# pierotofy/OpenSplat

Hardware: NVIDIA H100
Metric: fwd_bwd_mpixel_per_s (higher is better)
Workload: dtype f32

## Files before the change

include/gsplat_b200.h:

```cpp
#ifndef GSPLAT_B200_H
#define GSPLAT_B200_H

#include <stddef.h>
#include <stdint.h>

#ifdef __cplusplus
extern "C" {
#endif

#define GSB_TILE 16
#define GSB_ERR_INVALID_ARG (-1)
#define GSB_ERR_WORKSPACE (-2)
#define GSB_ERR_UNSUPPORTED (-3)
#define GSB_RASTER_CLAMP_MAX_ONE 1u
#define GSB_BIN_COUNT_VISIBLE 2

typedef void *gsb_stream_t;

int gsb_version(void);
const char *gsb_last_error(void);

int gsb_sh_forward(int n, int degree, int degrees_to_use, const float *viewdirs, const float *coeffs,
                   float *colors, gsb_stream_t stream);
int gsb_sh_backward(int n, int degree, int degrees_to_use, const float *viewdirs, const float *v_colors,
// ... 54 lines not shown
int gsb_project_backward_activated(int n, const float *means3d, const float *log_scales, float glob_scale,
                                   const float *raw_quats, const float *opacities, const float *viewmat,
                                   const float *projmat, float fx, float fy, int img_h, int img_w,
                                   const int32_t *radii, const float *conics, const float *v_xy,
                                   const float *v_depth, const float *v_conic, const float *v_opacity,
                                   float *v_mean3d, float *v_log_scales, float *v_raw_quats,
                                   float *v_opacity_logits, gsb_stream_t stream);
int gsb_project_backward_activated_acc(int n, const float *means3d, const float *log_scales, float glob_scale,
                                       const float *raw_quats, const float *opacities, const float *viewmat,
                                       const float *projmat, float fx, float fy, int img_h, int img_w,
                                       const int32_t *radii, const float *conics, const float *v_xy,
                                       const float *v_depth, const float *v_conic, const float *v_opacity,
                                       float *v_mean3d, float *v_log_scales, float *v_raw_quats,
                                       float *v_opacity_logits, gsb_stream_t stream);

size_t gsb_cumsum_workspace_bytes(int n);
int gsb_cumsum_tiles_hit(int n, const int32_t *num_tiles_hit, int32_t *cum_tiles_hit, void *workspace,
                         size_t workspace_bytes, gsb_stream_t stream);
int gsb_map_gaussian_to_intersects(int n, int m, const float *xys, const float *depths,
                                   const int32_t *radii, const int32_t *cum_tiles_hit, int tiles_x,
                                   int tiles_y, int64_t *isect_ids, int32_t *gaussian_ids,
                                   gsb_stream_t stream);
size_t gsb_sort_workspace_bytes(int m);
int gsb_sort_intersects(int m, int num_tiles, const int64_t *isect_ids, int64_t *isect_ids_sorted,
                        int32_t *sorted_index, void *workspace, size_t workspace_bytes,
                        gsb_stream_t stream);
int gsb_gather_bin_edges(int m, int num_tiles, const int64_t *isect_ids_sorted,
                         const int32_t *sorted_index, const int32_t *gaussian_ids,
                         int32_t *gaussian_ids_sorted, int32_t *tile_bins, gsb_stream_t stream);

int gsb_bucket_max_tile_len(void);
size_t gsb_bucket_workspace_bytes(int n, int m_capacity, int num_tiles);
int gsb_bucket_tile_ranges(int n, const float *xys, const int32_t *radii, const float *conics, const float *colors,
                           const float *opacities, int cull, int tiles_x, int tiles_y, int m_capacity,
                           int len_capacity, void *workspace, size_t workspace_bytes, int32_t *cum_tiles_hit,
                           int32_t *tile_bins, int32_t *tile_order, int32_t *stats, gsb_stream_t stream);
int gsb_bucket_sort_pack(int n, int m_capacity, int len_capacity, const float *depths, const int32_t *radii,
                         const int32_t *cum_tiles_hit, int cull, int tiles_x, int tiles_y, const int32_t *tile_bins,
                         const int32_t *stats, void *workspace, size_t workspace_bytes, void *records,
                         int32_t *sorted_index, int32_t *gaussian_ids_sorted, gsb_stream_t stream);

size_t gsb_raster_records_bytes(int m);
size_t gsb_raster_grad_rows_bytes(int m);
int gsb_pack_records(int m, const int32_t *gaussian_ids_sorted, const int32_t *sorted_index, const float *xys,
                     const float *conics, const float *colors, const float *opacities, void *records,
                     gsb_stream_t stream);
int gsb_rasterize_forward_packed(int img_h, int img_w, int tiles_x, int tiles_y, int m, const int32_t *tile_bins,
                                 const int32_t *tile_order, const int32_t *bin_stats, const float *background,
                                 void *records, float *out_img, float *final_Ts, int32_t *final_idx,
                                 unsigned flags, gsb_stream_t stream);
int gsb_rasterize_forward_count(int img_h, int img_w, int tiles_x, int tiles_y, int m, const int32_t *tile_bins,
                                const float *background, void *records, float *out_img, float *final_Ts,
                                int32_t *final_idx, unsigned long long *pair_counts, gsb_stream_t stream);
int gsb_rasterize_backward(int img_h, int img_w, int tiles_x, int tiles_y, int n, int m, const int32_t *tile_bins,
                           const int32_t *tile_order, const float *conics, const float *opacities, void *records,
                           const int32_t *cum_tiles_hit, const float *background, const float *final_Ts,
                           const int32_t *final_idx, const float *v_output, const float *v_output_alpha,
                           void *grad_rows, float *v_xy, float *v_conic, float *v_colors, float *v_opacity,
                           unsigned flags, gsb_stream_t stream);

int gsb_mse_loss_grad(long long n, const float *img, const float *target, float *v_img, float *loss_out,
                      float inv_count, gsb_stream_t stream);
int gsb_adam_step(long long n, float *param, const float *grad, float *exp_avg, float *exp_avg_sq, float lr,
                  float beta1, float beta2, float eps, float bias_correction1, float bias_correction2,
                  gsb_stream_t stream);
#define GSB_ADAM_MAX_SEGMENTS 8
typedef struct gsb_adam_segment {
    long long offset, count;
    int row_floats, head_floats;
    float lr_head, lr_rest;
} gsb_adam_segment;
int gsb_adam_step_segments(int num_segments, const gsb_adam_segment *segments, float *param, const float *grad,
                           float *exp_avg, float *exp_avg_sq, float beta1, float beta2, float eps,
                           float bias_correction1, float bias_correction2, gsb_stream_t stream);

int gsb_activate_forward(int n, const float *means, const float *log_scales, const float *raw_quats,
                         const float *opacity_logits, const float *cam_pos, float *scales, float *quats,
                         float *opacities, float *viewdirs, gsb_stream_t stream);
int gsb_activate_backward(int n, const float *scales, const float *raw_quats, const float *opacities,
                          const float *v_scales, const float *v_quats, const float *v_opacities,
                          float *v_log_scales, float *v_raw_quats, float *v_opacity_logits, gsb_stream_t stream);

int gsb_densify_stats_update(int n, const float *v_xy, const int32_t *radii, int img_h, int img_w,
                             float *xys_grad_norm, float *vis_counts, float *max_2d_size, gsb_stream_t stream);
int gsb_densify_stats_init(int n, const float *v_xy, const int32_t *radii, int img_h, int img_w,
                           float *xys_grad_norm, float *vis_counts, float *max_2d_size, gsb_stream_t stream);

size_t gsb_densify_workspace_bytes(int n);
int gsb_densify_classify(int n, const float *scales, const float *opacities, const float *xys_grad_norm,
                         const float *vis_counts, const float *max_2d_size, float max_dim,
                         float densify_grad_thresh, float densify_size_thresh, int check_split_screen,
                         float split_screen_size, float cull_alpha_thresh, int check_huge, float cull_scale_thresh,
                         int check_cull_screen, float cull_screen_size, float size_fac, void *workspace,
                         size_t workspace_bytes, int32_t *src_map, int32_t *split_rank, int32_t *counts,
                         gsb_stream_t stream);
int gsb_densify_means_scales(int new_n, int n_splits, const int32_t *src_map, const int32_t *split_rank,
                             const float *samples, const float *means, const float *scales, const float *quats,
                             float size_fac, float *new_means, float *new_scales, gsb_stream_t stream);
int gsb_densify_gather_rows(int new_n, int row_floats, const int32_t *src_map, const float *src, float *dst,
                            int zero_children, gsb_stream_t stream);
int gsb_reset_opacity(int n, float max_logit, float *opacities, float *exp_avg, float *exp_avg_sq,
                      gsb_stream_t stream);

int gsb_ply_row_floats(int sh_bases);
int gsb_pack_ply_rows(int n, int sh_bases, const float *means, const float *features_dc, int dc_stride,
                      const float *features_rest, int rest_stride, const float *opacities, const float *scales,
// ... 34 lines not shown
```

opensplat_b200/capi.py:

```python
import ctypes as C
import os

import torch

_HERE = os.path.dirname(os.path.abspath(__file__))
LIB_PATH = os.environ.get("GSB_LIB") or os.path.join(_HERE, "lib", "libgsplat_b200.so")
_lib = None

_vp, _i, _f, _sz = C.c_void_p, C.c_int, C.c_float, C.c_size_t

_SIGS = {
    "gsb_version": (C.c_int, []),
    "gsb_last_error": (C.c_char_p, []),
    "gsb_sh_forward": (_i, [_i, _i, _i, _vp, _vp, _vp, _vp]),
    "gsb_sh_backward": (_i, [_i, _i, _i, _vp, _vp, _vp, _vp]),
    "gsb_sh_forward_rgb": (_i, [_i, _i, _i, _vp, _vp, _f, _vp, _vp]),
    "gsb_sh_backward_rgb": (_i, [_i, _i, _i, _vp, _vp, _vp, _vp, _vp]),
    "gsb_sh_forward_split": (_i, [_i, _i, _i, _vp, _vp, _vp, _vp, _f, _vp, _vp]),
    "gsb_sh_backward_split": (_i, [_i, _i, _i, _vp, _vp, _vp, _vp, _vp, _vp, _vp]),
    "gsb_sh_forward_rgb_cam": (_i, [_i, _i, _i, _vp, _vp, _vp, _f, _vp, _vp]),
    "gsb_sh_backward_rgb_cam": (_i, [_i, _i, _i, _vp, _vp, _vp, _vp, _vp, _vp]),
    "gsb_sh_forward_rgb_cam_multiview": (_i, [_i, _i, _i, _vp, _i, _vp, _vp, _f, _vp, _vp]),
    "gsb_mask_rgb_grad": (_i, [_i, _vp, _vp, _vp]),
    "gsb_sh_backward_multiview": (_i, [_i, _i, _i, _vp, _i, _vp, _vp, _f, _vp, _vp]),
    "gsb_exchange_gradients": (_i, [_i, _i, _i, _vp, _i, _vp, _vp, _f, _vp, _i, _i, C.c_longlong, _vp, _vp, _vp]),
    "gsb_sh_backward_multiview_cams": (_i, [_i, _i, _i, _vp, _i, _vp, _vp, _f, _vp, _vp]),
    "gsb_exchange_gradients_cams": (_i, [_i, _i, _i, _vp, _i, _vp, _vp, _f, _vp, _i, _i, C.c_longlong, _vp, _vp,
                                         _vp]),
    "gsb_project_forward": (_i, [_i, _vp, _vp, _f, _vp, _vp, _vp, _f, _f, _f, _f, _i, _i, _i, _i, _f,
                                 _vp, _vp, _vp, _vp, _vp, _vp, _vp]),
    "gsb_project_backward": (_i, [_i, _vp, _vp, _f, _vp, _vp, _vp, _f, _f, _f, _f, _i, _i,
                                  _vp, _vp, _vp, _vp, _vp, _vp, _vp, _vp, _vp, _vp]),
    "gsb_project_forward_activated": (_i, [_i, _vp, _vp, _f, _vp, _vp, _vp, _vp, _f, _f, _f, _f, _i, _i, _i, _i, _f,
                                           _vp, _vp, _vp, _vp, _vp, _vp, _vp, _vp]),
    "gsb_project_backward_activated": (_i, [_i, _vp, _vp, _f, _vp, _vp, _vp, _vp, _f, _f, _i, _i,
                                            _vp, _vp, _vp, _vp, _vp, _vp, _vp, _vp, _vp, _vp, _vp]),
    "gsb_project_backward_activated_acc": (_i, [_i, _vp, _vp, _f, _vp, _vp, _vp, _vp, _f, _f, _i, _i,
                                                _vp, _vp, _vp, _vp, _vp, _vp, _vp, _vp, _vp, _vp, _vp]),
    "gsb_cumsum_workspace_bytes": (_sz, [_i]),
    "gsb_cumsum_tiles_hit": (_i, [_i, _vp, _vp, _vp, _sz, _vp]),
    "gsb_map_gaussian_to_intersects": (_i, [_i, _i, _vp, _vp, _vp, _vp, _i, _i, _vp, _vp, _vp]),
    "gsb_sort_workspace_bytes": (_sz, [_i]),
    "gsb_sort_intersects": (_i, [_i, _i, _vp, _vp, _vp, _vp, _sz, _vp]),
    "gsb_gather_bin_edges": (_i, [_i, _i, _vp, _vp, _vp, _vp, _vp, _vp]),
    "gsb_raster_records_bytes": (_sz, [_i]),
    "gsb_raster_grad_rows_bytes": (_sz, [_i]),
    "gsb_pack_records": (_i, [_i, _vp, _vp, _vp, _vp, _vp, _vp, _vp, _vp]),
    "gsb_rasterize_forward_packed": (_i, [_i, _i, _i, _i, _i, _vp, _vp, _vp, _vp, _vp, _vp, _vp, _vp, C.c_uint, _vp]),
    "gsb_rasterize_forward_count": (_i, [_i, _i, _i, _i, _i, _vp, _vp, _vp, _vp, _vp, _vp, _vp, _vp]),
    "gsb_rasterize_backward": (_i, [_i, _i, _i, _i, _i, _i, _vp, _vp, _vp, _vp, _vp, _vp, _vp, _vp, _vp, _vp,
                                    _vp, _vp, _vp, _vp, _vp, _vp, C.c_uint, _vp]),
    "gsb_bucket_max_tile_len": (_i, []),
    "gsb_bucket_workspace_bytes": (_sz, [_i, _i, _i]),
    "gsb_bucket_tile_ranges": (_i, [_i, _vp, _vp, _vp, _vp, _vp, _i, _i, _i, _i, _i, _vp, _sz, _vp, _vp, _vp, _vp, _vp]),
    "gsb_bucket_sort_pack": (_i, [_i, _i, _i, _vp, _vp, _vp, _i, _i, _i, _vp, _vp, _vp, _sz, _vp, _vp, _vp, _vp]),
    "gsb_activate_forward": (_i, [_i, _vp, _vp, _vp, _vp, _vp, _vp, _vp, _vp, _vp, _vp]),
    "gsb_activate_backward": (_i, [_i, _vp, _vp, _vp, _vp, _vp, _vp, _vp, _vp, _vp, _vp]),
    "gsb_densify_stats_update": (_i, [_i, _vp, _vp, _i, _i, _vp, _vp, _vp, _vp]),
    "gsb_densify_stats_init": (_i, [_i, _vp, _vp, _i, _i, _vp, _vp, _vp, _vp]),
    "gsb_densify_workspace_bytes": (_sz, [_i]),
    "gsb_densify_classify": (_i, [_i, _vp, _vp, _vp, _vp, _vp, _f, _f, _f, _i, _f, _f, _i, _f, _i, _f, _f, _vp, _sz,
                                  _vp, _vp, _vp, _vp]),
    "gsb_densify_means_scales": (_i, [_i, _i, _vp, _vp, _vp, _vp, _vp, _vp, _f, _vp, _vp, _vp]),
    "gsb_densify_gather_rows": (_i, [_i, _i, _vp, _vp, _vp, _i, _vp]),
    "gsb_reset_opacity": (_i, [_i, _f, _vp, _vp, _vp, _vp]),
    "gsb_ply_row_floats": (_i, [_i]),
    "gsb_pack_ply_rows": (_i, [_i, _i, _vp, _vp, _i, _vp, _i, _vp, _vp, _vp, _i, _f, C.POINTER(C.c_float), _vp, _vp]),
    "gsb_unpack_ply_rows": (_i, [_i, _i, _vp, _i, _f, C.POINTER(C.c_float), _vp, _vp, _i, _vp, _i, _vp, _vp, _vp, _vp]),
    "gsb_splat_order_keys": (_i, [_i, _vp, _vp, _i, _f, _vp, _vp]),
    "gsb_pack_splat_rows": (_i, [_i, _vp, _vp, _vp, _vp, _i, _vp, _vp, _i, _f, C.POINTER(C.c_float), _vp, _vp]),
    "gsb_ssim_workspace_bytes": (_sz, [_i, _i]),
    "gsb_ssim_l1_loss": (_i, [_i, _i, _vp, _vp, _f, _vp, _vp, _vp, _sz, _vp]),
    "gsb_adam_step": (_i, [C.c_longlong, _vp, _vp, _vp, _vp, _f, _f, _f, _f, _f, _f, _vp]),
    "gsb_adam_step_segments": (_i, [_i, _vp, _vp, _vp, _vp, _vp, _f, _f, _f, _f, _f, _vp]),
    "gsb_mse_loss_grad": (_i, [C.c_longlong, _vp, _vp, _vp, _vp, _f, _vp]),
    "gsb_knn_workspace_bytes": (_sz, [_i]),
    "gsb_knn_mean_dist": (_i, [_i, _vp, _vp, _vp, _sz, _vp]),
    "gsb_resize_area_u8": (_i, [_i, _i, _vp, _i, _i, _vp, _f, _vp]),
    "gsb_undistort_u8": (_i, [_i, _i, _vp, _f, _f, _f, _f, _f, _f, _f, _f, _f, _f, _f, _f, _f, _i, _i, _i, _i, _vp,
                              _vp]),
    "gsb_u8_to_f32_views": (_i, [_i, _vp, _i, _i, _vp, _vp]),
}

ADAM_MAX_SEGMENTS = 8


class AdamSegment(C.Structure):
    _fields_ = [("offset", C.c_longlong), ("count", C.c_longlong), ("row_floats", C.c_int),
                ("head_floats", C.c_int), ("lr_head", C.c_float), ("lr_rest", C.c_float)]
_OPT_SIGS = {}


class GsbError(RuntimeError):
    pass


def lib():
    global _lib
    if _lib is None:
        if not os.path.exists(LIB_PATH):
            raise GsbError(f"{LIB_PATH} not built -- run `python -m opensplat_b200.build` "
                           "(there is no CPU fallback)")
# ... 38 lines not shown
```

opensplat_b200/csrc/bucket.cu:

```cuda
#include "raster_common.cuh"

namespace {

constexpr int CUR_STRIDE = 32;
constexpr int BIN_THREADS = 256;
constexpr int TSCAN_THREADS = 1024;

constexpr int LEN_BUCKETS = 64;
struct BinHeader {
    unsigned ticket_n;
    unsigned ticket_t;
    unsigned done_t;
    int max_len;
    int total;
    int visible;
    int pad0[2];
    int len_hist[LEN_BUCKETS];
    int len_cur[LEN_BUCKETS];
    int pad[120];
};
static_assert(sizeof(BinHeader) == 1024, "header is 1 KB");

__device__ __forceinline__ int len_bucket(int v, int len_capacity) {
    const long long b = (long long)v * LEN_BUCKETS / ((long long)max(len_capacity, 1) + 1);
// ... 16 lines not shown
    if (blk == 0) {
        if (lane == 0) st_state(&state[0], ST_INC | (unsigned)aggregate);
        return 0;
    }
    if (lane == 0) st_state(&state[blk], ST_AGG | (unsigned)aggregate);
    int excl = 0;
    int j = blk - 1;
    while (true) {
        const int idx = j - lane;
        unsigned long long s = ST_INC;
        if (idx >= 0) s = ld_state(&state[idx]);
        const unsigned flag = (unsigned)(s >> 62);
        if (__ballot_sync(0xffffffffu, flag == 0u)) continue;
        const unsigned incm = __ballot_sync(0xffffffffu, flag == 2u);
        int val = (int)(unsigned)(s & ST_VAL);
        if (incm) {
            const int first = __ffs(incm) - 1;
            if (lane > first) val = 0;
            excl += __reduce_add_sync(0xffffffffu, val);
            break;
        }
        excl += __reduce_add_sync(0xffffffffu, val);
        j -= 32;
    }
    if (lane == 0) st_state(&state[blk], ST_INC | (unsigned)(excl + aggregate));
    return excl;
}

__global__ void __launch_bounds__(BIN_THREADS)
bin_count_kernel(int n, const float2 *__restrict__ xys, const int *__restrict__ radii,
                 const float *__restrict__ conics, const float *__restrict__ colors,
                 const float *__restrict__ opacities, int cull, int tiles_x, int tiles_y,
                 int *__restrict__ tile_count, GsbRecord *__restrict__ gattr, int *__restrict__ count_out,
                 int *__restrict__ visible) {
    const int i = blockIdx.x * BIN_THREADS + threadIdx.x;
    const int r = (i < n) ? radii[i] : 0;
    if (visible) {
        const int nvis = __syncthreads_count(r > 0);
        if (threadIdx.x == 0 && nvis > 0) atomicAdd(visible, nvis);
    }
    if (i >= n) return;
    int cnt = 0;
    if (r > 0) {
        const float2 c = xys[i];
        const GsbRecord rec = make_record(c, __ldg(conics + 3 * i), __ldg(conics + 3 * i + 1),
                                          __ldg(conics + 3 * i + 2), __ldg(opacities + i), __ldg(colors + 3 * i),
                                          __ldg(colors + 3 * i + 1), __ldg(colors + 3 * i + 2), 0);
        float4 *dst = reinterpret_cast<float4 *>(gattr + i);
        dst[0] = rec.q0; dst[1] = rec.q1; dst[2] = rec.q2;
        int x0, x1, y0, y1;
        gsb_tile_bbox(c.x, c.y, (float)r, tiles_x, tiles_y, x0, x1, y0, y1);
        for (int ty = y0; ty < y1; ++ty)
            for (int tx = x0; tx < x1; ++tx) {
                if (cull && !extent_slot_mask(c.x, c.y, rec.q1.w, rec.q2.w, (float)(tx * GSB_TILE),
                                              (float)(ty * GSB_TILE)))
                    continue;
                atomicAdd(&tile_count[(size_t)(ty * tiles_x + tx) * CUR_STRIDE], 1);
                ++cnt;
            }
    }
    count_out[i] = cnt;
}

constexpr int GS_IPT = 8;
__global__ void __launch_bounds__(BIN_THREADS)
count_scan_kernel(int n, int *__restrict__ counts_then_cum, unsigned *ticket, unsigned long long *state) {
    __shared__ int sm[BIN_THREADS / 32 + 1];
    __shared__ int s_blk, s_prefix;
    if (threadIdx.x == 0) s_blk = (int)atomicAdd(ticket, 1u);
    __syncthreads();
    const int blk = s_blk;
    const int e0 = (blk * BIN_THREADS + threadIdx.x) * GS_IPT;
    int v[GS_IPT];
    const bool vec = (e0 + GS_IPT <= n) && ((reinterpret_cast<uintptr_t>(counts_then_cum + e0) & 15) == 0);
    if (vec) {
        const int4 a = *reinterpret_cast<const int4 *>(counts_then_cum + e0);
        const int4 b = *reinterpret_cast<const int4 *>(counts_then_cum + e0 + 4);
        v[0] = a.x; v[1] = a.y; v[2] = a.z; v[3] = a.w; v[4] = b.x; v[5] = b.y; v[6] = b.z; v[7] = b.w;
    } else {
#pragma unroll
        for (int k = 0; k < GS_IPT; ++k) v[k] = (e0 + k < n) ? counts_then_cum[e0 + k] : 0;
    }
    int tsum = 0;
#pragma unroll
    for (int k = 0; k < GS_IPT; ++k) tsum += v[k];
    int total;
    int run = block_excl_scan<BIN_THREADS>(tsum, &total, sm);
    if (threadIdx.x < 32) {
        const int p = chained_scan_prefix(state, blk, total);
        if (threadIdx.x == 0) s_prefix = p;
    }
    __syncthreads();
    run += s_prefix;
#pragma unroll
    for (int k = 0; k < GS_IPT; ++k) { run += v[k]; v[k] = run; }
    if (vec) {
        *reinterpret_cast<int4 *>(counts_then_cum + e0) = make_int4(v[0], v[1], v[2], v[3]);
        *reinterpret_cast<int4 *>(counts_then_cum + e0 + 4) = make_int4(v[4], v[5], v[6], v[7]);
    } else {
#pragma unroll
        for (int k = 0; k < GS_IPT; ++k)
            if (e0 + k < n) counts_then_cum[e0 + k] = v[k];
    }
}

}

int gsb_count_scan_blocks(int n) { return gsb_div_up(n > 0 ? n : 1, BIN_THREADS * GS_IPT); }
// ... 23 lines not shown
        const int p = chained_scan_prefix(state, blk, total);
        if (threadIdx.x == 0) s_prefix = p;
    }
    __syncthreads();
    if (t < T) {
        const int e = s_prefix + excl;
        tile_bins[t] = (v > 0) ? make_int2(e, e + v) : make_int2(0, 0);
        tile_count_then_cursor[(size_t)t * CUR_STRIDE] = e;
    }
    if (threadIdx.x == 0) {
        if (s_max > 0) atomicMax(&hdr->max_len, s_max);
        if (blk == nblk - 1) atomicExch(&hdr->total, s_prefix + total);
        __threadfence();
        const unsigned done = atomicAdd(&hdr->done_t, 1u);
        if (done == (unsigned)nblk - 1u) {
            __threadfence();
            const int M = atomicAdd(&hdr->total, 0), mx = atomicAdd(&hdr->max_len, 0);
            stats[0] = M;
            stats[1] = mx;
            stats[2] = (M > m_capacity || mx > len_capacity) ? 1 : 0;
            stats[3] = hdr->visible;
        }
    }
}

__global__ void __launch_bounds__(TSCAN_THREADS)
tile_order_kernel(int T, int len_capacity, BinHeader *hdr, const int2 *__restrict__ tile_bins,
                  int *__restrict__ tile_order) {
    __shared__ int base[LEN_BUCKETS];
    if (threadIdx.x < LEN_BUCKETS) {
        int sfx = 0;
        for (int b = LEN_BUCKETS - 1; b > (int)threadIdx.x; --b) sfx += hdr->len_hist[b];
        base[threadIdx.x] = sfx;
    }
    __syncthreads();
    const int t = blockIdx.x * TSCAN_THREADS + threadIdx.x;
    if (t >= T) return;
    const int2 r = tile_bins[t];
    const int b = len_bucket(r.y - r.x, len_capacity);
    tile_order[base[b] + atomicAdd(&hdr->len_cur[b], 1)] = t;
}

__global__ void __launch_bounds__(256)
bucket_emit_kernel(int n, const GsbRecord *__restrict__ gattr, const float *__restrict__ depths,
                   const int *__restrict__ radii, const int *__restrict__ cum_tiles_hit, int cull, int tiles_x,
                   int tiles_y, int *__restrict__ cursor, unsigned long long *__restrict__ comp,
                   int *__restrict__ gaussian_ids, int *__restrict__ gid_at_pos, const int *__restrict__ stats) {
    if (stats[2]) return;
    const int i = blockIdx.x * blockDim.x + threadIdx.x;
    if (i >= n) return;
    const int r = radii[i];
    if (r <= 0) return;
    const float4 *src = reinterpret_cast<const float4 *>(gattr + i);
    const float4 q0 = src[0];
    const float hx = src[1].w, hy = src[2].w;
    int x0, x1, y0, y1;
    gsb_tile_bbox(q0.x, q0.y, (float)r, tiles_x, tiles_y, x0, x1, y0, y1);
    int k = (i == 0) ? 0 : cum_tiles_hit[i - 1];
    const unsigned long long hi = ((unsigned long long)(unsigned)__float_as_int(depths[i])) << 32;
    for (int ty = y0; ty < y1; ++ty)
        for (int tx = x0; tx < x1; ++tx) {
            if (cull && !extent_slot_mask(q0.x, q0.y, hx, hy, (float)(tx * GSB_TILE), (float)(ty * GSB_TILE)))
                continue;
            const int pos = atomicAdd(&cursor[(size_t)(ty * tiles_x + tx) * CUR_STRIDE], 1);
            comp[pos] = hi | (unsigned)k;
            if (gid_at_pos) gid_at_pos[pos] = i;
            gaussian_ids[k] = i;
            ++k;
        }
}

typedef unsigned long long u64;

constexpr int DS_MIN_BINS = 64, DS_MAX_BINS = 2048;
constexpr int DS_BIN_LIMIT = 32;

constexpr int BITONIC_MAX = 4096;

__device__ __forceinline__ u64 shfl_xor_u64(u64 v, int m) {
    unsigned lo = (unsigned)v, hi = (unsigned)(v >> 32);
    lo = __shfl_xor_sync(0xffffffffu, lo, m);
    hi = __shfl_xor_sync(0xffffffffu, hi, m);
    return ((u64)hi << 32) | lo;
}

__device__ __forceinline__ u64 cex_shfl(u64 v, int j, bool keep_min) {
    const u64 o = shfl_xor_u64(v, j);
    return ((v < o) == keep_min) ? v : o;
}

__device__ __forceinline__ void block64_substages(u64 &a, u64 &b, int base, int lane, int k, int jstart) {
    const int ia = base + lane, ib = ia + 32;
    const bool asc_a = (ia & k) == 0, asc_b = (ib & k) == 0;
    if (jstart >= 32) {
        const bool sw = (a > b) == asc_a;
        const u64 t = sw ? b : a;
        b = sw ? a : b;
        a = t;
    }
#pragma unroll
    for (int j = 16; j >= 1; j >>= 1) {
        if (j > jstart) continue;
        const bool lower = (lane & j) == 0;
        a = cex_shfl(a, j, lower == asc_a);
        b = cex_shfl(b, j, lower == asc_b);
    }
}

template <int ITEMS>
__device__ __forceinline__ void cta_radix_sort_depth(u64 *buf, unsigned (*whist)[256], unsigned *bin_base,
                                                    unsigned *s_flag) {
    const int lane = threadIdx.x & 31, w = threadIdx.x >> 5;
    const int wbase = w * 32 * ITEMS;
    u64 key[ITEMS];
    unsigned rank[ITEMS];
// ... 480 lines not shown
```

opensplat_b200/csrc/raster_bwd.cu:

```cuda
#include "raster_common.cuh"

int gsb_blend_grid(const void *kernel, int num_tiles);

namespace {

__device__ __forceinline__ float rcp_approx(float x) {
    float y;
    asm("rcp.approx.ftz.f32 %0, %1;" : "=f"(y) : "f"(x));
    return y;
}

__device__ __forceinline__ void zero_row(float *grad_rows, int k) {
    float4 *row = reinterpret_cast<float4 *>(grad_rows + (size_t)k * GSB_GRAD_ROW_FLOATS);
    const float4 z = make_float4(0.f, 0.f, 0.f, 0.f);
    row[0] = z; row[1] = z; row[2] = z;
}

constexpr int BWD_MIN_BLOCKS = 6;
template <bool SAT>
__global__ void __launch_bounds__(RK_THREADS, BWD_MIN_BLOCKS)
rasterize_backward_kernel(int img_h, int img_w, int tiles_x, int num_tiles,
                          const int2 *__restrict__ tile_bins, const GsbRecord *__restrict__ records,
                          const float *__restrict__ background, const float *__restrict__ final_Ts,
                          const int *__restrict__ final_idx, const float *__restrict__ v_output,
                          const float *__restrict__ v_output_alpha, float *__restrict__ grad_rows,
                          unsigned *__restrict__ tile_counter, const int *__restrict__ tile_order) {
    __shared__ WarpRing rings[RK_WARPS];
    const int warp = threadIdx.x >> 5, lane = threadIdx.x & 31;
    WarpRing &ring = rings[warp];
    if (lane == 0) {
#pragma unroll
        for (int s = 0; s < RK_STAGES; ++s) mbar_init(&ring.full[s], 1);
        mbar_fence_init();
    }
    __syncwarp();
    const float bg0 = __ldg(background), bg1 = __ldg(background + 1), bg2 = __ldg(background + 2);
    unsigned gchunk = 0;

    while (true) {
        int tile = 0;
        if (lane == 0) tile = (int)atomicAdd(tile_counter, 1u);
        tile = __shfl_sync(0xffffffffu, tile, 0);
        if (tile >= num_tiles) break;
        if (tile_order) tile = __ldg(tile_order + tile);
        const int2 range = tile_bins[tile];
        if (range.y <= range.x) continue;

        const int tx = tile % tiles_x, ty = tile / tiles_x;
        const int X = tx * GSB_TILE + (lane & 15);
        const int Y0 = ty * GSB_TILE + (lane >> 4);
        const float px = (float)X;
        const float tile_x0 = (float)(tx * GSB_TILE), tile_y0 = (float)(ty * GSB_TILE);

        float T[RK_PIX], Bq[RK_PIX];
        const float py0 = (float)Y0;
        float vor[RK_PIX], vog[RK_PIX], vob[RK_PIX];
        int binf[RK_PIX];
        int my_max = -1;
#pragma unroll
        for (int j = 0; j < RK_PIX; ++j) {
            const int Y = Y0 + 2 * j;
            if (X < img_w && Y < img_h) {
                const size_t p = (size_t)Y * img_w + X;
// ... 227 lines not shown
```

opensplat_b200/csrc/raster_common.cuh:

```cuda
#pragma once
#include "gsb_common.cuh"

struct __align__(16) GsbRecord {
    float4 q0, q1, q2;
};
static_assert(sizeof(GsbRecord) == 48, "record must be 48 bytes");

constexpr int RK_WARPS = 4;
constexpr int RK_THREADS = RK_WARPS * 32;
constexpr int RK_PIX = 8;
constexpr int RK_CHUNK = 32;
constexpr int RK_STAGES = 4;

constexpr float GSB_LN2 = 0.6931471805599453f;
constexpr float GSB_LOG2E = 1.4426950408889634f;
constexpr float GSB_SMAX_BIAS = 5.541263545158426f + 1e-3f;

constexpr int GSB_GRAD_ROW_FLOATS = 12;

constexpr int GSB_SAT_BIT0 = 1 << 28;
constexpr int GSB_SAT_MASK = 7 << 28;

struct __align__(128) WarpRing {
    GsbRecord rec[RK_STAGES][RK_CHUNK];
    uint64_t full[RK_STAGES];
};

#ifdef __CUDACC__
__device__ __forceinline__ GsbRecord make_record(float2 xy, float a, float b, float c, float opac, float r,
                                                 float g, float bl, int k) {
    const float lo = (opac > 0.f) ? log2f(opac) : -INFINITY;
    const float smax = fmaxf(0.f, fmaf(lo, GSB_LN2, GSB_SMAX_BIAS));
    const float det = a * c - b * b;
    float hx = INFINITY, hy = INFINITY;
    if (det > 0.f && a > 0.f && c > 0.f) {
        const float s2 = 2.f * smax / det;
        hx = sqrtf(s2 * c) * 1.001f + 0.01f;
        hy = sqrtf(s2 * a) * 1.001f + 0.01f;
    }
    GsbRecord rec;
    rec.q0 = make_float4(xy.x, xy.y, lo, __int_as_float(k));
    rec.q1 = make_float4(0.5f * a, b, 0.5f * c, hx);
    rec.q2 = make_float4(r, g, bl, hy);
    return rec;
}

__device__ __forceinline__ unsigned extent_slot_mask(float cx, float cy, float hx, float hy, float tile_x0,
                                                     float tile_y0) {
    const float gx = cx - tile_x0, gy = cy - tile_y0;
    const float xlo = fmaxf(ceilf(gx - hx), 0.f), xhi = fminf(floorf(gx + hx), 15.f);
    const float ylo = fmaxf(ceilf(gy - hy), 0.f), yhi = fminf(floorf(gy + hy), 15.f);
    if (!(xlo <= xhi) || !(ylo <= yhi)) return 0u;
    const int jlo = (int)ylo >> 1, jhi = (int)yhi >> 1;
    return ((2u << jhi) - 1u) & ~((1u << jlo) - 1u);
}

__device__ __forceinline__ unsigned record_slot_mask(const GsbRecord &r, float tile_x0, float tile_y0) {
    return extent_slot_mask(r.q0.x, r.q0.y, r.q1.w, r.q2.w, tile_x0, tile_y0);
}
#endif
```

opensplat_b200/csrc/raster_fwd.cu:

```cuda
#include "raster_common.cuh"

namespace {

__global__ void __launch_bounds__(256)
pack_records_kernel(int m, const int *__restrict__ gaussian_ids_sorted,
                    const int *__restrict__ sorted_index, const float2 *__restrict__ xys,
                    const float *__restrict__ conics, const float *__restrict__ colors,
                    const float *__restrict__ opacities, GsbRecord *__restrict__ records) {
    const int i = blockIdx.x * blockDim.x + threadIdx.x;
    if (i >= m) return;
    const int g = gaussian_ids_sorted[i];
    const int k = sorted_index ? sorted_index[i] : i;
    const GsbRecord r = make_record(__ldg(xys + g), __ldg(conics + 3 * g), __ldg(conics + 3 * g + 1),
                                    __ldg(conics + 3 * g + 2), __ldg(opacities + g), __ldg(colors + 3 * g),
                                    __ldg(colors + 3 * g + 1), __ldg(colors + 3 * g + 2), k);
    float4 *dst = reinterpret_cast<float4 *>(records + i);
    stg_stream4(dst, r.q0);
    stg_stream4(dst + 1, r.q1);
    stg_stream4(dst + 2, r.q2);
}

constexpr int FWD_MIN_BLOCKS = 8;
template <bool COUNT, bool SAT>
__global__ void __launch_bounds__(RK_THREADS, FWD_MIN_BLOCKS)
rasterize_forward_kernel(int img_h, int img_w, int tiles_x, int num_tiles,
                         const int2 *__restrict__ tile_bins, const GsbRecord *__restrict__ records,
                         const float *__restrict__ background, float *__restrict__ out_img,
                         float *__restrict__ final_Ts, int *__restrict__ final_idx,
                         unsigned *__restrict__ tile_counter, const int *__restrict__ bin_stats,
                         unsigned long long *__restrict__ pair_counts, const int *__restrict__ tile_order) {
    if (bin_stats && bin_stats[2]) return;
    __shared__ WarpRing rings[RK_WARPS];
    const int warp = threadIdx.x >> 5, lane = threadIdx.x & 31;
    WarpRing &ring = rings[warp];
    if (lane == 0) {
#pragma unroll
        for (int s = 0; s < RK_STAGES; ++s) mbar_init(&ring.full[s], 1);
        mbar_fence_init();
    }
    __syncwarp();
    const float bg0 = __ldg(background), bg1 = __ldg(background + 1), bg2 = __ldg(background + 2);
    unsigned gchunk = 0;
    unsigned long long n_rec = 0, n_slot = 0, n_eval = 0, n_blend = 0;

    while (true) {
        int tile = 0;
        if (lane == 0) tile = (int)atomicAdd(tile_counter, 1u);
        tile = __shfl_sync(0xffffffffu, tile, 0);
        if (tile >= num_tiles) break;
        if (tile_order) tile = __ldg(tile_order + tile);

        const int tx = tile % tiles_x, ty = tile / tiles_x;
        const int X = tx * GSB_TILE + (lane & 15);
        const int Y0 = ty * GSB_TILE + (lane >> 4);
        const float px = (float)X;
        const float tile_x0 = (float)(tx * GSB_TILE), tile_y0 = (float)(ty * GSB_TILE);
        const int2 range = tile_bins[tile];
        const int L = range.y - range.x;
        const int nchunks = (L + RK_CHUNK - 1) / RK_CHUNK;

        float T[RK_PIX], cr[RK_PIX], cg[RK_PIX], cb[RK_PIX];
        const float py0 = (float)Y0;
        int last[RK_PIX];
        unsigned done = 0;
#pragma unroll
        for (int j = 0; j < RK_PIX; ++j) {
            T[j] = 1.f; cr[j] = cg[j] = cb[j] = 0.f; last[j] = 0;
            if (X >= img_w || Y0 + 2 * j >= img_h) { done |= 1u << j; T[j] = -1.f; }
        }

        const unsigned g0 = gchunk;
        auto stage_of = [&](int c) { return (g0 + (unsigned)c) % RK_STAGES; };
        auto parity_of = [&](int c) { return ((g0 + (unsigned)c) / RK_STAGES) & 1u; };
        auto issue = [&](int c) {
            if (lane == 0) {
                const int cnt = min(RK_CHUNK, L - c * RK_CHUNK);
                const uint32_t bytes = (uint32_t)cnt * (uint32_t)sizeof(GsbRecord);
                const unsigned s = stage_of(c);
                mbar_arrive_expect_tx(&ring.full[s], bytes);
                tma_load_1d(&ring.rec[s][0], records + range.x + c * RK_CHUNK, bytes, &ring.full[s]);
            }
        };
        const int pro = min(RK_STAGES, nchunks);
        for (int c = 0; c < pro; ++c) issue(c);
        int issued = pro;

        int c = 0;
        for (; c < nchunks; ++c) {
            const unsigned s = stage_of(c);
            mbar_wait(&ring.full[s], parity_of(c));
            const int cnt = min(RK_CHUNK, L - c * RK_CHUNK);
            const int idx0 = range.x + c * RK_CHUNK;
            unsigned my_mask = 0;
            if (lane < cnt) my_mask = record_slot_mask(ring.rec[s][lane], tile_x0, tile_y0);
            unsigned live = __ballot_sync(0xffffffffu, my_mask != 0u);
            if (COUNT && lane == 0) n_rec += __popc(live);
            while (live) {
                const int t = __ffs(live) - 1;
                live &= live - 1;
                const unsigned rm = __shfl_sync(0xffffffffu, my_mask, t);
                const float4 q0 = ring.rec[s][t].q0;
                const float4 q1 = ring.rec[s][t].q1;
                const float4 q2 = ring.rec[s][t].q2;
                const float smax = fmaxf(0.f, fmaf(q0.z, GSB_LN2, GSB_SMAX_BIAS));
                const float dx = q0.x - px;
                const float adx2 = q1.x * dx * dx;
                const float bdx = q1.y * dx;
                const float dy0 = q0.y - py0;
                const int idx = idx0 + t;
                const int jhi = 31 - __clz(rm);
#define GSB_FWD_SLOT(j)                                                                                   \
    {                                                                                                     \
        const float dy = dy0 - (float)(2 * j);                                                                      \
                                      \
        const float sigma = fmaf(dy, fmaf(q1.z, dy, bdx), adx2);                                          \
        if (COUNT && lane == 0) ++n_slot;                                                                 \
        if (__float_as_uint(sigma) <= __float_as_uint(smax)) {            \
                     \
            const float alpha = fminf(0.999f, ex2_approx(fmaf(sigma, -GSB_LOG2E, q0.z)));                 \
            if (COUNT) ++n_eval;                                                                          \
            if (alpha >= (1.f / 255.f)) {                                                                 \
                const float next_T = T[j] * (1.f - alpha);                                                \
                if (next_T <= 1e-4f) {                                     \
                    if (T[j] > 0.f) { T[j] = -T[j]; done |= 1u << j; }                                    \
                } else {                                                                                  \
                    const float vis = alpha * T[j];                                                       \
                    cr[j] = fmaf(q2.x, vis, cr[j]);                                                       \
                    cg[j] = fmaf(q2.y, vis, cg[j]);                                                       \
                    cb[j] = fmaf(q2.z, vis, cb[j]);                                                       \
                    T[j] = next_T;                                                                        \
                    last[j] = idx;                                                                        \
                    if (COUNT) ++n_blend;                                                                 \
                }                                                                                         \
            }                                                                                             \
        }                                                                                                 \
        if (jhi == j) break;                                                                              \
    }
                do {
                    if (rm & 1u) GSB_FWD_SLOT(0)
                    if (rm & 2u) GSB_FWD_SLOT(1)
                    if (rm & 4u) GSB_FWD_SLOT(2)
                    if (rm & 8u) GSB_FWD_SLOT(3)
                    if (rm & 16u) GSB_FWD_SLOT(4)
                    if (rm & 32u) GSB_FWD_SLOT(5)
                    if (rm & 64u) GSB_FWD_SLOT(6)
                    if (rm & 128u) GSB_FWD_SLOT(7)
                } while (0);
#undef GSB_FWD_SLOT
            }
            if (__all_sync(0xffffffffu, done == 0xffu)) { ++c; break; }
            __syncwarp();
            if (issued < nchunks) { issue(issued); ++issued; }
        }
        for (; c < issued; ++c) mbar_wait(&ring.full[stage_of(c)], parity_of(c));
        gchunk = g0 + (unsigned)issued;
        __syncwarp();

#pragma unroll
        for (int j = 0; j < RK_PIX; ++j) {
            const int Y = Y0 + 2 * j;
            if (X < img_w && Y < img_h) {
                const size_t p = (size_t)Y * img_w + X;
                const float Tf = fabsf(T[j]);
                final_Ts[p] = Tf;
                float o0 = cr[j] + Tf * bg0, o1 = cg[j] + Tf * bg1, o2 = cb[j] + Tf * bg2;
                int fi = last[j];
                if (SAT) {
                    if (!(o0 <= 1.f)) { fi |= GSB_SAT_BIT0; o0 = o0 > 1.f ? 1.f : o0; }
                    if (!(o1 <= 1.f)) { fi |= GSB_SAT_BIT0 << 1; o1 = o1 > 1.f ? 1.f : o1; }
                    if (!(o2 <= 1.f)) { fi |= GSB_SAT_BIT0 << 2; o2 = o2 > 1.f ? 1.f : o2; }
                }
                final_idx[p] = fi;
                out_img[3 * p] = o0;
                out_img[3 * p + 1] = o1;
                out_img[3 * p + 2] = o2;
            }
        }
    }
    if (COUNT) {
        n_eval = __reduce_add_sync(0xffffffffu, (unsigned)n_eval);
        n_blend = __reduce_add_sync(0xffffffffu, (unsigned)n_blend);
        if (lane == 0) {
            atomicAdd(pair_counts + 0, n_rec);
            atomicAdd(pair_counts + 1, n_slot);
            atomicAdd(pair_counts + 2, n_eval);
            atomicAdd(pair_counts + 3, n_blend);
        }
    }
}


}

int gsb_sm_count();
int gsb_blend_grid(const void *kernel, int num_tiles);

extern "C" size_t gsb_raster_records_bytes(int m) {
    return gsb_align_up((size_t)(m > 0 ? m : 0) * sizeof(GsbRecord), 256) + 256;
}

// ... 19 lines not shown
    GSB_CHECK_ARG(tile_bins && background && out_img && final_Ts && final_idx && records);
    GSB_CHECK_ARG(((uintptr_t)records % 16) == 0);
    *counters = reinterpret_cast<unsigned *>(reinterpret_cast<char *>(records) + gsb_raster_records_bytes(m) - 256);
    GSB_CUDA(cudaMemsetAsync(*counters, 0, 256, s));
    return 0;
}

extern "C" int gsb_rasterize_forward_packed(int img_h, int img_w, int tiles_x, int tiles_y, int m,
                                            const int32_t *tile_bins, const int32_t *tile_order,
                                            const int32_t *bin_stats, const float *background, void *records,
                                            float *out_img, float *final_Ts, int32_t *final_idx, unsigned flags,
                                            gsb_stream_t stream) {
    GSB_CHECK_ARG((flags & ~(unsigned)GSB_RASTER_CLAMP_MAX_ONE) == 0);
    const bool sat = (flags & GSB_RASTER_CLAMP_MAX_ONE) != 0;
    GSB_CHECK_ARG(!sat || m < GSB_SAT_BIT0);
    cudaStream_t s = (cudaStream_t)stream;
    unsigned *counters = nullptr;
    const int rc = blend_setup(img_h, img_w, tiles_x, tiles_y, m, tile_bins, background, records, out_img, final_Ts,
                               final_idx, s, &counters);
    if (rc) return rc;
    const int num_tiles = tiles_x * tiles_y;
#define GSB_FWD_LAUNCH(S)                                                                                        \
    rasterize_forward_kernel<false, S><<<gsb_blend_grid((const void *)rasterize_forward_kernel<false, S>, num_tiles), \
                                         RK_THREADS, 0, s>>>(                                                    \
        img_h, img_w, tiles_x, num_tiles, reinterpret_cast<const int2 *>(tile_bins),                             \
        reinterpret_cast<const GsbRecord *>(records), background, out_img, final_Ts, final_idx, counters,        \
        bin_stats, nullptr, tile_order)
    if (sat) GSB_FWD_LAUNCH(true); else GSB_FWD_LAUNCH(false);
#undef GSB_FWD_LAUNCH
    GSB_LAUNCH_CHECK();
    return 0;
}

extern "C" int gsb_rasterize_forward_count(int img_h, int img_w, int tiles_x, int tiles_y, int m,
                                           const int32_t *tile_bins, const float *background, void *records,
                                           float *out_img, float *final_Ts, int32_t *final_idx,
                                           unsigned long long *pair_counts, gsb_stream_t stream) {
    GSB_CHECK_ARG(pair_counts);
    cudaStream_t s = (cudaStream_t)stream;
    unsigned *counters = nullptr;
    const int rc = blend_setup(img_h, img_w, tiles_x, tiles_y, m, tile_bins, background, records, out_img, final_Ts,
                               final_idx, s, &counters);
    if (rc) return rc;
    const int num_tiles = tiles_x * tiles_y;
    const int grid = gsb_blend_grid((const void *)rasterize_forward_kernel<true, false>, num_tiles);
    rasterize_forward_kernel<true, false><<<grid, RK_THREADS, 0, s>>>(
        img_h, img_w, tiles_x, num_tiles, reinterpret_cast<const int2 *>(tile_bins),
        reinterpret_cast<const GsbRecord *>(records), background, out_img, final_Ts, final_idx, counters, nullptr,
        pair_counts, nullptr);
    GSB_LAUNCH_CHECK();
    return 0;
}

int gsb_sm_count() {
    static thread_local int cached_dev = -1, cached = 0;
    int dev = 0;
    cudaGetDevice(&dev);
    if (dev != cached_dev) {
        cudaDeviceGetAttribute(&cached, cudaDevAttrMultiProcessorCount, dev);
        if (cached <= 0) cached = 132;
        cached_dev = dev;
    }
    return cached;
}

int gsb_blend_grid(const void *kernel, int num_tiles) {
    struct Entry { const void *kernel; int dev; int per_sm; };
    static thread_local Entry cache[8] = {};
    int dev = 0;
    cudaGetDevice(&dev);
    int per_sm = 0;
    for (const Entry &e : cache)
        if (e.kernel == kernel && e.dev == dev) per_sm = e.per_sm;
    if (per_sm == 0) {
        if (cudaOccupancyMaxActiveBlocksPerMultiprocessor(&per_sm, kernel, RK_THREADS, 0) != cudaSuccess || per_sm < 1)
            per_sm = 1;
        for (Entry &e : cache)
            if (e.kernel == nullptr || e.kernel == kernel) { e = Entry{kernel, dev, per_sm}; break; }
    }
    const int full = gsb_sm_count() * per_sm;
    const int need = gsb_div_up(num_tiles, RK_WARPS);
    return need < full ? need : full;
}
```

Measured before the change: 1090.

## Cull tile-gaussian pairs and row slots using exact ellipse extent

```diff
diff --git a/include/gsplat_b200.h b/include/gsplat_b200.h
--- a/include/gsplat_b200.h
+++ b/include/gsplat_b200.h
@@ -130,6 +130,8 @@
 int gsb_rasterize_forward_count(int img_h, int img_w, int tiles_x, int tiles_y, int m, const int32_t *tile_bins,
                                 const float *background, void *records, float *out_img, float *final_Ts,
                                 int32_t *final_idx, unsigned long long *pair_counts, gsb_stream_t stream);
+int gsb_record_slot_masks(int m, const void *records, const int32_t *tiles, int tiles_x, uint8_t *masks,
+                          gsb_stream_t stream);
 int gsb_rasterize_backward(int img_h, int img_w, int tiles_x, int tiles_y, int n, int m, const int32_t *tile_bins,
                            const int32_t *tile_order, const float *conics, const float *opacities, void *records,
                            const int32_t *cum_tiles_hit, const float *background, const float *final_Ts,
diff --git a/opensplat_b200/capi.py b/opensplat_b200/capi.py
--- a/opensplat_b200/capi.py
+++ b/opensplat_b200/capi.py
@@ -48,6 +48,7 @@
     "gsb_pack_records": (_i, [_i, _vp, _vp, _vp, _vp, _vp, _vp, _vp, _vp]),
     "gsb_rasterize_forward_packed": (_i, [_i, _i, _i, _i, _i, _vp, _vp, _vp, _vp, _vp, _vp, _vp, _vp, C.c_uint, _vp]),
     "gsb_rasterize_forward_count": (_i, [_i, _i, _i, _i, _i, _vp, _vp, _vp, _vp, _vp, _vp, _vp, _vp]),
+    "gsb_record_slot_masks": (_i, [_i, _vp, _vp, _i, _vp, _vp]),
     "gsb_rasterize_backward": (_i, [_i, _i, _i, _i, _i, _i, _vp, _vp, _vp, _vp, _vp, _vp, _vp, _vp, _vp, _vp,
                                     _vp, _vp, _vp, _vp, _vp, _vp, C.c_uint, _vp]),
     "gsb_bucket_max_tile_len": (_i, []),
diff --git a/opensplat_b200/csrc/bucket.cu b/opensplat_b200/csrc/bucket.cu
--- a/opensplat_b200/csrc/bucket.cu
+++ b/opensplat_b200/csrc/bucket.cu
@@ -92,8 +92,8 @@
         gsb_tile_bbox(c.x, c.y, (float)r, tiles_x, tiles_y, x0, x1, y0, y1);
         for (int ty = y0; ty < y1; ++ty)
             for (int tx = x0; tx < x1; ++tx) {
-                if (cull && !extent_slot_mask(c.x, c.y, rec.q1.w, rec.q2.w, (float)(tx * GSB_TILE),
-                                              (float)(ty * GSB_TILE)))
+                if (cull && !ellipse_slot_mask(c.x, c.y, rec.q1.x, rec.q1.y, rec.q1.z, rec.q1.w, rec.q2.w, rec.q0.z,
+                                               (float)(tx * GSB_TILE), (float)(ty * GSB_TILE)))
                     continue;
                 atomicAdd(&tile_count[(size_t)(ty * tiles_x + tx) * CUR_STRIDE], 1);
                 ++cnt;
@@ -223,15 +223,16 @@
     const int r = radii[i];
     if (r <= 0) return;
     const float4 *src = reinterpret_cast<const float4 *>(gattr + i);
-    const float4 q0 = src[0];
-    const float hx = src[1].w, hy = src[2].w;
+    const float4 q0 = src[0], q1 = src[1];
+    const float hy = src[2].w;
     int x0, x1, y0, y1;
     gsb_tile_bbox(q0.x, q0.y, (float)r, tiles_x, tiles_y, x0, x1, y0, y1);
     int k = (i == 0) ? 0 : cum_tiles_hit[i - 1];
     const unsigned long long hi = ((unsigned long long)(unsigned)__float_as_int(depths[i])) << 32;
     for (int ty = y0; ty < y1; ++ty)
         for (int tx = x0; tx < x1; ++tx) {
-            if (cull && !extent_slot_mask(q0.x, q0.y, hx, hy, (float)(tx * GSB_TILE), (float)(ty * GSB_TILE)))
+            if (cull && !ellipse_slot_mask(q0.x, q0.y, q1.x, q1.y, q1.z, q1.w, hy, q0.z, (float)(tx * GSB_TILE),
+                                           (float)(ty * GSB_TILE)))
                 continue;
             const int pos = atomicAdd(&cursor[(size_t)(ty * tiles_x + tx) * CUR_STRIDE], 1);
             comp[pos] = hi | (unsigned)k;
diff --git a/opensplat_b200/csrc/raster_bwd.cu b/opensplat_b200/csrc/raster_bwd.cu
--- a/opensplat_b200/csrc/raster_bwd.cu
+++ b/opensplat_b200/csrc/raster_bwd.cu
@@ -3,12 +3,6 @@
 int gsb_blend_grid(const void *kernel, int num_tiles);
 
 namespace {
-
-__device__ __forceinline__ float rcp_approx(float x) {
-    float y;
-    asm("rcp.approx.ftz.f32 %0, %1;" : "=f"(y) : "f"(x));
-    return y;
-}
 
 __device__ __forceinline__ void zero_row(float *grad_rows, int k) {
     float4 *row = reinterpret_cast<float4 *>(grad_rows + (size_t)k * GSB_GRAD_ROW_FLOATS);
diff --git a/opensplat_b200/csrc/raster_common.cuh b/opensplat_b200/csrc/raster_common.cuh
--- a/opensplat_b200/csrc/raster_common.cuh
+++ b/opensplat_b200/csrc/raster_common.cuh
@@ -27,6 +27,17 @@
 };
 
 #ifdef __CUDACC__
+__device__ __forceinline__ float rcp_approx(float x) {
+    float y;
+    asm("rcp.approx.ftz.f32 %0, %1;" : "=f"(y) : "f"(x));
+    return y;
+}
+__device__ __forceinline__ float sqrt_approx(float x) {
+    float y;
+    asm("sqrt.approx.ftz.f32 %0, %1;" : "=f"(y) : "f"(x));
+    return y;
+}
+
 __device__ __forceinline__ GsbRecord make_record(float2 xy, float a, float b, float c, float opac, float r,
                                                  float g, float bl, int k) {
     const float lo = (opac > 0.f) ? log2f(opac) : -INFINITY;
@@ -45,17 +56,36 @@
     return rec;
 }
 
-__device__ __forceinline__ unsigned extent_slot_mask(float cx, float cy, float hx, float hy, float tile_x0,
-                                                     float tile_y0) {
-    const float gx = cx - tile_x0, gy = cy - tile_y0;
-    const float xlo = fmaxf(ceilf(gx - hx), 0.f), xhi = fminf(floorf(gx + hx), 15.f);
-    const float ylo = fmaxf(ceilf(gy - hy), 0.f), yhi = fminf(floorf(gy + hy), 15.f);
+__device__ __forceinline__ unsigned ellipse_slot_mask(float cx, float cy, float A, float B, float C, float hx,
+                                                      float hy, float lo, float tile_x0, float tile_y0) {
+    const float gx = __fsub_rn(cx, tile_x0), gy = __fsub_rn(cy, tile_y0);
+    const float xlo = fmaxf(ceilf(__fsub_rn(gx, hx)), 0.f), xhi = fminf(floorf(__fadd_rn(gx, hx)), 15.f);
+    float ylo = fmaxf(ceilf(__fsub_rn(gy, hy)), 0.f), yhi = fminf(floorf(__fadd_rn(gy, hy)), 15.f);
     if (!(xlo <= xhi) || !(ylo <= yhi)) return 0u;
+    const float bb = __fmul_rn(B, B);
+    const float det4 = __fsub_rn(__fmaf_rn(4.f * A, C, -bb), __fmaf_rn(B, B, -bb));
+    const float s = __fmul_rn(fmaxf(0.f, __fmaf_rn(lo, GSB_LN2, GSB_SMAX_BIAS)), 1.f + 1.f / 512.f);
+    const float ymax = sqrt_approx(__fmul_rn(__fmul_rn(4.f * A, s), rcp_approx(det4)));
+    const float r2a = rcp_approx(A + A), r2c = rcp_approx(C + C);
+    if (hx < INFINITY && det4 > 0.f && ymax < INFINITY && r2a < INFINITY && r2c < INFINITY) {
+        const float ex = __fmaf_rn(hx, 1.f / 512.f, 1.f / 64.f), ey = __fmaf_rn(hy, 1.f / 512.f, 1.f / 64.f);
+        const float Xl = __fsub_rn(__fsub_rn(gx, xhi), ex), Xr = __fadd_rn(__fsub_rn(gx, xlo), ex);
+        const float xt = __fmul_rn(__fmul_rn(-B, r2a), ymax);
+        const float C4s = __fmul_rn(4.f * C, s);
+        const float Xh = fminf(fmaxf(xt, Xl), Xr), Xb = fminf(fmaxf(-xt, Xl), Xr);
+        const float wh = sqrt_approx(fmaxf(0.f, __fmaf_rn(-det4, __fmul_rn(Xh, Xh), C4s)));
+        const float wb = sqrt_approx(fmaxf(0.f, __fmaf_rn(-det4, __fmul_rn(Xb, Xb), C4s)));
+        const float dhi = (Xh == xt) ? ymax : __fmul_rn(__fmaf_rn(-B, Xh, wh), r2c);
+        const float dlo = (Xb == -xt) ? -ymax : __fmul_rn(__fmaf_rn(-B, Xb, -wb), r2c);
+        ylo = fmaxf(ylo, ceilf(__fsub_rn(__fsub_rn(gy, dhi), ey)));
+        yhi = fminf(yhi, floorf(__fadd_rn(__fsub_rn(gy, dlo), ey)));
+        if (!(ylo <= yhi)) return 0u;
+    }
     const int jlo = (int)ylo >> 1, jhi = (int)yhi >> 1;
     return ((2u << jhi) - 1u) & ~((1u << jlo) - 1u);
 }
 
 __device__ __forceinline__ unsigned record_slot_mask(const GsbRecord &r, float tile_x0, float tile_y0) {
-    return extent_slot_mask(r.q0.x, r.q0.y, r.q1.w, r.q2.w, tile_x0, tile_y0);
+    return ellipse_slot_mask(r.q0.x, r.q0.y, r.q1.x, r.q1.y, r.q1.z, r.q1.w, r.q2.w, r.q0.z, tile_x0, tile_y0);
 }
 #endif
diff --git a/opensplat_b200/csrc/raster_fwd.cu b/opensplat_b200/csrc/raster_fwd.cu
--- a/opensplat_b200/csrc/raster_fwd.cu
+++ b/opensplat_b200/csrc/raster_fwd.cu
@@ -18,6 +18,16 @@
     stg_stream4(dst, r.q0);
     stg_stream4(dst + 1, r.q1);
     stg_stream4(dst + 2, r.q2);
+}
+
+__global__ void __launch_bounds__(256)
+record_slot_masks_kernel(int m, const GsbRecord *__restrict__ records, const int *__restrict__ tiles, int tiles_x,
+                         unsigned char *__restrict__ masks) {
+    const int i = blockIdx.x * blockDim.x + threadIdx.x;
+    if (i >= m) return;
+    const int t = tiles[i];
+    masks[i] = (unsigned char)record_slot_mask(records[i], (float)(t % tiles_x * GSB_TILE),
+                                               (float)(t / tiles_x * GSB_TILE));
 }
 
 constexpr int FWD_MIN_BLOCKS = 8;
@@ -108,7 +118,7 @@
                 const float bdx = q1.y * dx;
                 const float dy0 = q0.y - py0;
                 const int idx = idx0 + t;
-                const int jhi = 31 - __clz(rm);
+                const int jlo = __ffs(rm) - 1, jhi = 31 - __clz(rm);
 #define GSB_FWD_SLOT(j)                                                                                   \
     {                                                                                                     \
         const float dy = dy0 - (float)(2 * j);                                                                      \
@@ -136,16 +146,16 @@
         }                                                                                                 \
         if (jhi == j) break;                                                                              \
     }
-                do {
-                    if (rm & 1u) GSB_FWD_SLOT(0)
-                    if (rm & 2u) GSB_FWD_SLOT(1)
-                    if (rm & 4u) GSB_FWD_SLOT(2)
-                    if (rm & 8u) GSB_FWD_SLOT(3)
-                    if (rm & 16u) GSB_FWD_SLOT(4)
-                    if (rm & 32u) GSB_FWD_SLOT(5)
-                    if (rm & 64u) GSB_FWD_SLOT(6)
-                    if (rm & 128u) GSB_FWD_SLOT(7)
-                } while (0);
+                switch (jlo) {
+                    case 0: GSB_FWD_SLOT(0)
+                    case 1: GSB_FWD_SLOT(1)
+                    case 2: GSB_FWD_SLOT(2)
+                    case 3: GSB_FWD_SLOT(3)
+                    case 4: GSB_FWD_SLOT(4)
+                    case 5: GSB_FWD_SLOT(5)
+                    case 6: GSB_FWD_SLOT(6)
+                    default: GSB_FWD_SLOT(7)
+                }
 #undef GSB_FWD_SLOT
             }
             if (__all_sync(0xffffffffu, done == 0xffu)) { ++c; break; }
@@ -271,6 +281,17 @@
     return 0;
 }
 
+extern "C" int gsb_record_slot_masks(int m, const void *records, const int32_t *tiles, int tiles_x, uint8_t *masks,
+                                     gsb_stream_t stream) {
+    GSB_CHECK_ARG(m >= 0 && tiles_x > 0);
+    if (m == 0) return 0;
+    GSB_CHECK_ARG(records && tiles && masks && ((uintptr_t)records % 16) == 0);
+    record_slot_masks_kernel<<<gsb_div_up(m, 256), 256, 0, (cudaStream_t)stream>>>(
+        m, reinterpret_cast<const GsbRecord *>(records), tiles, tiles_x, masks);
+    GSB_LAUNCH_CHECK();
+    return 0;
+}
+
 int gsb_sm_count() {
     static thread_local int cached_dev = -1, cached = 0;
     int dev = 0;
```

After: 1114 (median of 6 runs). 1.02x the previous value.
